# microscopic-image-analysis/DiffPointRasterisation.jl

Hardware: AMD Instinct MI355X
Metric: M points/s fwd+bwd, 10M pts→256³ grid; HBM GB/s vs roofline (higher is better)
Workload: dtype f32

## Files before the change

diffpointrasterisation.jl_amd/csrc/dpr_tiled.hip:

```cpp
#include <hip/hip_runtime.h>

#include <cstring>
#include <mutex>
#include <set>
#include <type_traits>
#include <utility>

#include "dpr_tiled_impl.h"

namespace dpr {

template <int NO>
__device__ __forceinline__ int primary_tile(const int (&ref0)[NO], const TileGeom<NO>& tg) {
    int t = 0, stride = 1;
    bool in = true;
#pragma unroll
    for (int d = 0; d < NO; ++d) {
        const int r = ref0[d] < 0 ? 0 : ref0[d];
        int c = r / TileDims<NO>::T[d];
        if (d == NO - 1) {
            c -= tg.tz0;
            in = (unsigned)c < (unsigned)tg.nt[d];
        }
        t += c * stride;
// ... 506 lines not shown
    __syncthreads();
    const Pose<T, NI, NO> ps = load_pose<T, NI, NO>(rot, trans, nullptr, b);
    const int64_t lo = (int64_t)slice * chunk;
    const int64_t hi = (lo + chunk < P) ? lo + chunk : P;
    if (lo >= hi) return;
    uint32_t wkey = 0;
    int64_t p = lo + threadIdx.x;
    T nxt[NI], nxt_w = T(1);
    {
        const int64_t pl = p < hi ? p : hi - 1;
        load_point<T, NI>(points, pl, nxt);
        if (HAS_PW) nxt_w = pw[pl];
    }
#pragma unroll
    for (int j = 0; j < NI; ++j) pin_value(nxt[j]);
    if (HAS_PW) pin_value(nxt_w);
    drain_vmem();
    while (p < hi) {
        T pt[NI];
#pragma unroll
        for (int j = 0; j < NI; ++j) pt[j] = nxt[j];
        const T w = nxt_w;
        const int64_t pc = p;
        p += kBinThreads;
        {
            const int64_t pl = p < hi ? p : hi - 1;
            load_point<T, NI>(points, pl, nxt);
            if (HAS_PW) nxt_w = pw[pl];
        }
        int ref0[NO];
        T dlo[NO];
        bool valid = ref_and_deltas<T, NI, NO>(pt, ps, gd, ref0, dlo);
        const int tl = valid ? primary_tile<NO>(ref0, tg) : -1;
        valid = tl >= 0;
        uint32_t pos = (uint32_t)P;
        if (valid) pos = atomicAdd(&cursor[tl], 1u);
        if (HAS_PW && valid) wkey = wrange_merge(wkey, abs_key(w));
        Rec4<T> r;
#pragma unroll
        for (int j = 0; j < 3; ++j) r.v[j] = (j < NI) ? pt[(j < NI) ? j : 0] : T(0);
        r.v[3] = HAS_PW ? w : idx_to_slot((uint32_t)pc, T(0));
        rec[pos] = r;
        if (HAS_PW && WANT_IDX) rec_idx[pos] = (uint32_t)pc;
        if (WANT_IDX) slot_of[pc] = pos;
        if (zero_dropped && !valid) {
#pragma unroll
            for (int j = 0; j < NI; ++j) ds_dpoints[pc * NI + j] = T(0);
            if (ds_dpw) ds_dpw[pc] = T(0);
        }
    }
    if (HAS_PW) publish_max_abs(maxpw, wkey);
}

template <typename T, int NI, int NO, bool HAS_PW, int S, bool GROUP, bool W3>
__global__ __launch_bounds__(kWcThreads) void k_scatter_wc(
    GridDesc<NO> gd, TileGeom<NO> tg, int64_t P, int64_t chunk, const T* __restrict__ points,
    const T* __restrict__ pw, const T* __restrict__ rot, const T* __restrict__ trans, int64_t b0,
    int nb, const uint32_t* __restrict__ prefix, const uint32_t* __restrict__ tile_start,
    RecT<T, W3>* __restrict__ rec, uint32_t* __restrict__ slot_of, T* __restrict__ ds_dpoints,
    T* __restrict__ ds_dpw, int zero_dropped, uint32_t* __restrict__ maxpw, int fused_scan,
    TileScanArgs ts) {
    const unsigned n_slices = fused_scan ? gridDim.x - 1u : gridDim.x;
    if (fused_scan && blockIdx.x == n_slices) {
        tilescan_body(ts.totals, ts.NT, ts.cap, ts.tile_start, ts.items, ts.n_items, ts.tile_parts,
                      ts.tile_slab, ts.split_list, ts.n_split, ts.hdr, ts.hdr_out, ts.rot,
                      ts.rot_words, ts.trans, ts.trans_words, ts.nonzero_bins, ts.nblk);
        return;
    }
    static_assert(!(W3 && HAS_PW), "compact records carry no point weight");
    constexpr int PPT = S / kWcThreads;
    uint32_t wkey = 0;
    if (!GROUP) nb = 1;
    const int NT = tg.NT, NTe = NT * nb;
    const uint32_t Pe = (uint32_t)(P * nb);
    extern __shared__ uint32_t dyn[];
    uint32_t* cursor = dyn;
    uint32_t* lhist = dyn + NTe;
    __shared__ RecT<T, W3> recs[S];
    __shared__ uint32_t dest[S];
    uint32_t* const wsum = dest;
    static_assert(S >= kWcThreads / kWave, "wave sums fit");
    const unsigned slice = xcd_slice(blockIdx.x, n_slices);
    const uint32_t* row = prefix + (size_t)slice * NTe;
    constexpr int kMaxBpt = 4096 / kWcThreads;
    const int lane = threadIdx.x & (kWave - 1), wave = threadIdx.x / kWave;
    if (fused_scan) {
        const int bpe = (NTe + kWcThreads - 1) / kWcThreads;
        const int e0 = threadIdx.x * bpe;
        uint32_t c[kMaxBpt], rw[kMaxBpt], sum = 0;
#pragma unroll
        for (int q = 0; q < kMaxBpt; ++q) {
            const int i = e0 + q;
            const bool in = q < bpe && i < NTe;
            c[q] = in ? ts.totals[i] : 0u;
            rw[q] = in ? row[i] : 0u;
            sum += c[q];
        }
        uint32_t incl = sum;
#pragma unroll
        for (int o = 1; o < kWave; o <<= 1) {
            const uint32_t v = __shfl_up(incl, o, kWave);
            if (lane >= o) incl += v;
        }
        if (lane == kWave - 1) wsum[wave] = incl;
        __syncthreads();
        uint32_t run = incl - sum;
        for (int wv = 0; wv < wave; ++wv) run += wsum[wv];
#pragma unroll
        for (int q = 0; q < kMaxBpt; ++q) {
            const int i = e0 + q;
            if (q < bpe && i < NTe) cursor[i] = run + rw[q];
            run += c[q];
        }
    } else {
        for (int i = threadIdx.x; i < NTe; i += kWcThreads) cursor[i] = tile_start[i] + row[i];
    }
    for (int i = threadIdx.x; i < NT; i += kWcThreads) lhist[i] = 0;
    __syncthreads();
    const int64_t lo = (int64_t)slice * chunk;
    const int64_t hi = (lo + chunk < P) ? lo + chunk : P;
    const int bpt = (NT + kWcThreads - 1) / kWcThreads;
    const int bin0 = threadIdx.x * bpt;
    if (lo >= hi) return;
    constexpr bool kPrefetch = !GROUP;
    auto load_sub = [&](int64_t sbase, T (&dp)[PPT][NI], T (&dw)[PPT]) {
        const int64_t left = hi - sbase;
        const uint32_t n = left >= S ? (uint32_t)S : (left > 0 ? (uint32_t)left : 0u);
        const T* const pb = points + (n ? sbase : hi - 1) * NI;
        const T* const wb = HAS_PW ? pw + (n ? sbase : hi - 1) : nullptr;
#pragma unroll
        for (int k = 0; k < PPT; ++k) {
            const uint32_t lp = threadIdx.x + (uint32_t)k * kWcThreads;
// ... 27 lines not shown
#pragma unroll
            for (int k = 0; k < PPT; ++k) {
                const uint32_t lp = threadIdx.x + (uint32_t)k * kWcThreads;
                int ref0[NO];
                T dlo[NO];
                bool valid = ref_and_deltas<T, NI, NO>(pt[k], ps, gd, ref0, dlo) && lp < nloc;
                tile[k] = valid ? primary_tile<NO>(ref0, tg) : -1;
                valid = tile[k] >= 0;
                lrank[k] = 0;
                if (valid) lrank[k] = atomicAdd(&lhist[tile[k]], 1u);
                if (HAS_PW && valid) wkey = wrange_merge(wkey, abs_key(w[k]));
            }
            lds_barrier();
            uint32_t cnt_sum = 0;
            uint32_t cnt[kMaxBpt];
#pragma unroll
            for (int q = 0; q < kMaxBpt; ++q) {
                const int i = bin0 + q;
                cnt[q] = (q < bpt && i < NT) ? lhist[i] : 0u;
                cnt_sum += cnt[q];
            }
            uint32_t incl = cnt_sum;
#pragma unroll
            for (int o = 1; o < kWave; o <<= 1) {
                const uint32_t v = __shfl_up(incl, o, kWave);
                if (lane >= o) incl += v;
            }
            if (lane == kWave - 1) wsum[wave] = incl;
            lds_barrier();
            uint32_t run = incl - cnt_sum;
            for (int wv = 0; wv < wave; ++wv) run += wsum[wv];
            uint32_t n_valid = 0;
#pragma unroll
            for (int wv = 0; wv < kWcThreads / kWave; ++wv) n_valid += wsum[wv];
#pragma unroll
            for (int q = 0; q < kMaxBpt; ++q) {
                const int i = bin0 + q;
                if (q < bpt && i < NT) lhist[i] = run;
                run += cnt[q];
            }
            lds_barrier();
#pragma unroll
            for (int k = 0; k < PPT; ++k) {
                const uint32_t lp = threadIdx.x + (uint32_t)k * kWcThreads;
                if (tile[k] >= 0) {
                    const uint32_t sidx = lhist[tile[k]] + lrank[k];
                    const uint32_t d = cur[tile[k]] + lrank[k];
                    RecT<T, W3> r;
#pragma unroll
                    for (int j = 0; j < 3; ++j) r.v[j] = (j < NI) ? pt[k][(j < NI) ? j : 0] : T(0);
                    if constexpr (!W3) r.v[3] = HAS_PW ? w[k] : idx_to_slot((uint32_t)base + lp, T(0));
                    recs[sidx] = r;
                    dest[sidx] = d;
                    if (slot_b) __builtin_nontemporal_store(d, &slot_b[lp]);
                } else if (lp < nloc) {
                    if (slot_b) __builtin_nontemporal_store(Pe, &slot_b[lp]);
                    if (zero_dropped) {
                        T* const dp_b = ds_dpoints + base * NI;
#pragma unroll
                        for (int j = 0; j < NI; ++j) dp_b[lp * NI + j] = T(0);
                        if (ds_dpw) (ds_dpw + base)[lp] = T(0);
                    }
                }
            }
            lds_barrier();
            for (uint32_t i = threadIdx.x; i < n_valid; i += kWcThreads) rec[dest[i]] = recs[i];
#pragma unroll
            for (int q = 0; q < kMaxBpt; ++q) {
                const int i = bin0 + q;
                if (q < bpt && i < NT) {
                    cur[i] += cnt[q];
                    lhist[i] = 0;
                }
            }
            lds_barrier();
        }
    }
    if (HAS_PW) publish_max_abs(maxpw, wkey);
}

struct LocalBinArgs {
    char* ws;
    size_t pose_stride;
    size_t off_rec, off_slot, off_desc, off_bdesc, off_ltot;
};
constexpr int kTouchCap = 1024;
template <typename T, int NI, int NO, bool HAS_PW, int S, bool W3, bool ONE, int TH, bool STAGE>
__global__ __launch_bounds__(TH, ((sizeof(T) == 4 && ONE) ? 8 : 4)) void k_bin_local(
    GridDesc<NO> gd, TileGeom<NO> tg, int64_t P, const T* __restrict__ points,
    const T* __restrict__ pw, const T* __restrict__ rot, const T* __restrict__ trans, int64_t b0,
    int nb, LocalBinArgs la, int want_slot, uint32_t spare_slot, T* __restrict__ ds_dpoints,
    T* __restrict__ ds_dpw, int zero_dropped) {
    static_assert(!(W3 && HAS_PW), "compact records carry no point weight");
    constexpr int PPT = S / TH;
    if (ONE) nb = 1;
    const int NT = tg.NT;
    extern __shared__ uint32_t lhist[];
    __shared__ RecT<T, W3> recs[STAGE ? S : 1];
    __shared__ uint16_t touched[kTouchCap];
    __shared__ uint32_t wsum[TH / kWave];
    __shared__ uint32_t s_ntouch, s_nvalid;
    for (int i = threadIdx.x; i < NT; i += TH) lhist[i] = 0;
    if (threadIdx.x == 0) s_ntouch = 0;
    const int64_t base = (int64_t)blockIdx.x * S;
    const uint32_t nloc = (uint32_t)((P - base < S) ? P - base : S);
    const T* const pts_blk = points + base * NI;
    const T* const pw_blk = HAS_PW ? pw + base : nullptr;
    T pt[PPT][NI], w[PPT];
#pragma unroll
    for (int k = 0; k < PPT; ++k) {
        const uint32_t lp = threadIdx.x + (uint32_t)k * TH;
        const uint32_t ll = lp < nloc ? lp : nloc - 1;
        if (nloc) {
            load_point<T, NI>(pts_blk, (int64_t)ll, pt[k]);
            w[k] = HAS_PW ? pw_blk[ll] : T(1);
        } else {
#pragma unroll
            for (int j = 0; j < NI; ++j) pt[k][j] = T(0);
            w[k] = T(1);
        }
    }
    if constexpr (HAS_PW) {
        uint32_t wkey = 0;
#pragma unroll
        for (int k = 0; k < PPT; ++k)
            if (threadIdx.x + (uint32_t)k * TH < nloc) wkey = wrange_merge(wkey, abs_key(w[k]));
        publish_max_abs((uint32_t*)(la.ws + la.off_ltot) + 2 * NT, wkey);
    }
    __syncthreads();
    const int lane = threadIdx.x & (kWave - 1), wave = threadIdx.x / kWave;
#pragma unroll 1
// ... 1698 lines not shown
    if (stale) {
        const T nan = T(__builtin_nanf(""));
        const int64_t b0 = (int64_t)ublock * (kUPB * 1024) + threadIdx.x;
#pragma unroll
        for (int k = 0; k < kUPB; ++k) {
            const int64_t p = b0 + k * 1024;
            if (p >= P) continue;
#pragma unroll
            for (int j = 0; j < NI; ++j) ds_dpoints[p * NI + j] = nan;
            if (ds_dpw) ds_dpw[p] = nan;
        }
        return;
    }
    const int64_t base = (int64_t)xcd_slice(ublock, ublocks) * (kUPB * 1024) + threadIdx.x;
    uint32_t slot[kUPB];
#pragma unroll
    for (int k = 0; k < kUPB; ++k) {
        const int64_t p = base + k * 1024;
        slot[k] = __builtin_nontemporal_load(&slot_of[p < P ? p : P - 1]);
    }
    Rec4<T> g[kUPB];
#pragma unroll
    for (int k = 0; k < kUPB; ++k) g[k] = grad[slot[k]];
    for (int j = 1; j < nb; ++j) {
        const Rec4<T>* gradj =
            pose_stride ? (const Rec4<T>*)((const char*)grad + (size_t)j * pose_stride) : grad;
        const uint32_t* slotj = pose_stride
                                    ? (const uint32_t*)((const char*)slot_of + (size_t)j * pose_stride)
                                    : slot_of + (size_t)j * P;
#pragma unroll
        for (int k = 0; k < kUPB; ++k) {
            const int64_t p = base + k * 1024;
            const Rec4<T> gj = gradj[slotj[p < P ? p : P - 1]];
#pragma unroll
            for (int c = 0; c < 4; ++c) g[k].v[c] += gj.v[c];
        }
    }
#pragma unroll
    for (int k = 0; k < kUPB; ++k) {
        const int64_t p = base + k * 1024;
        if (p >= P) continue;
        if (FIRST_POSE) {
#pragma unroll
            for (int j = 0; j < NI; ++j) __builtin_nontemporal_store(g[k].v[j], &ds_dpoints[p * NI + j]);
            if (ds_dpw) __builtin_nontemporal_store(g[k].v[3], &ds_dpw[p]);
        } else {
#pragma unroll
            for (int j = 0; j < NI; ++j) ds_dpoints[p * NI + j] += g[k].v[j];
            if (ds_dpw) ds_dpw[p] += g[k].v[3];
        }
    }
}

template <typename T>
__global__ __launch_bounds__(1024) void k_pose_reduce(PoseReduceArgs<T> pr) {
    pose_reduce_body<T>((int)blockIdx.x, blockIdx.y, gridDim.y > 1, pr);
}

template <typename T, int NI>
__global__ __launch_bounds__(256) void k_unsort(int64_t P, const uint32_t* __restrict__ inv_perm,
                                                const T* __restrict__ dp_sorted,
                                                const T* __restrict__ dpw_sorted,
                                                T* __restrict__ ds_dpoints, T* __restrict__ ds_dpw,
                                                const BinHeader* __restrict__ hdr) {
    constexpr int PER = 4;
    const int64_t q0 = (int64_t)blockIdx.x * (256 * PER) + threadIdx.x;
    if (hdr && hdr->verdict != 1u) {
        const T nan = T(__builtin_nanf(""));
#pragma unroll
        for (int k = 0; k < PER; ++k) {
            const int64_t q = q0 + k * 256;
            if (q >= P) continue;
#pragma unroll
            for (int j = 0; j < NI; ++j) ds_dpoints[q * NI + j] = nan;
            if (ds_dpw) ds_dpw[q] = nan;
        }
        return;
    }
    size_t i[PER];
#pragma unroll
    for (int k = 0; k < PER; ++k) {
        const int64_t q = q0 + k * 256;
        const size_t v = inv_perm[q < P ? q : P - 1];
        i[k] = v < (size_t)P ? v : 0;
    }
    T v[PER][NI], w[PER];
#pragma unroll
    for (int k = 0; k < PER; ++k) {
#pragma unroll
        for (int j = 0; j < NI; ++j) v[k][j] = dp_sorted[i[k] * NI + j];
        w[k] = ds_dpw ? dpw_sorted[i[k]] : T(0);
    }
#pragma unroll
    for (int k = 0; k < PER; ++k) {
        const int64_t q = q0 + k * 256;
        if (q >= P) continue;
#pragma unroll
        for (int j = 0; j < NI; ++j) ds_dpoints[q * NI + j] = v[k][j];
        if (ds_dpw) ds_dpw[q] = w[k];
    }
}

static int cu_count() {
    static std::mutex mu;
    static int cus[64] = {0};
    int dev = 0;
// ... 41 lines not shown
        while (nb * 2 <= pl.bg && b + nb * 2 <= B) nb *= 2;
        return nb;
    }
    int64_t copy_of(int64_t b) const { return kept && B > 1 ? b : (pl.local ? b % pl.lb : 0); }
    PoseWs at(int64_t b) const { return {ws + (size_t)copy_of(b) * pl.pose_stride, pl}; }
    bool opens_local_batch(int64_t b) const { return b % pl.lb == 0; }
    int local_batch(int64_t b) const { return (int)((B - b < pl.lb) ? B - b : pl.lb); }
};

template <typename K> static int allow_dynamic_lds(K kernel, size_t bytes, int max_bytes) {
    if (bytes <= 48 * 1024) return DPR_OK;
    static std::mutex mu;
    static std::set<std::pair<const void*, int>> done;
    int dev = 0;
    DPR_HIP(hipGetDevice(&dev));
    std::lock_guard<std::mutex> lock(mu);
    if (done.count({(const void*)kernel, dev})) return DPR_OK;
    DPR_HIP(hipFuncSetAttribute((const void*)kernel, hipFuncAttributeMaxDynamicSharedMemorySize, max_bytes));
    done.insert({(const void*)kernel, dev});
    return DPR_OK;
}


static bool scatter_is_wc(int NT, int nb) { return NT * nb <= 4096; }

static bool records_are_compact(int NT, int nb, bool has_pw, bool want_idx) {
    return !has_pw && !want_idx && scatter_is_wc(NT, nb);
}

template <typename T, int NI, int NO, bool HAS_PW, bool WANT_IDX>
static int launch_scatter(hipStream_t st, const GridDesc<NO>& gd, const TileGeom<NO>& tg,
                          const Plan& pl, const PoseWs& w, int64_t P, const T* points, const T* pw,
                          const T* rot, const T* trans, int64_t b, int nb, const TileScanArgs& ts,
                          bool fused) {
    if (scatter_is_wc(tg.NT, nb)) {
        constexpr int S = (sizeof(T) == 4) ? kWcPpt * kWcThreads : kWcPpt * kWcThreads / 2;
        const size_t lds2 = (size_t)tg.NT * (nb + 1) * 4;
#define DPR_LAUNCH_WC(GROUP, W3)                                                                  \
    hipLaunchKernelGGL((k_scatter_wc<T, NI, NO, HAS_PW, S, GROUP, W3>),                          \
                       dim3(pl.nblk + (fused ? 1 : 0)),                                          \
                       dim3(kWcThreads), lds2, st, gd, tg, P, pl.chunk, points, pw, rot, trans, \
                       b, nb, w.counts(), w.tile_start(),      \
                       w.rec<RecT<T, W3>>(),                                                     \
                       WANT_IDX ? w.slot() : (uint32_t*)nullptr,                                 \
                       (T*)nullptr, (T*)nullptr, 0, w.weight_keys(), fused ? 1 : 0, ts)
        if constexpr (!HAS_PW) {
            if (records_are_compact(tg.NT, nb, false, WANT_IDX)) {
                if (nb > 1) DPR_LAUNCH_WC(true, true);
                else DPR_LAUNCH_WC(false, true);
                return DPR_OK;
            }
        }
        if (nb > 1) DPR_LAUNCH_WC(true, false);
        else DPR_LAUNCH_WC(false, false);
#undef DPR_LAUNCH_WC
        return DPR_OK;
    }
    const size_t lds = (size_t)tg.NT * 4;
    if (int rc = allow_dynamic_lds(k_scatter<T, NI, NO, HAS_PW, WANT_IDX>, lds, kMaxTiles * 4)) return rc;
    hipLaunchKernelGGL((k_scatter<T, NI, NO, HAS_PW, WANT_IDX>), dim3(pl.nblk), dim3(kBinThreads),
                       lds, st, gd, tg, P, pl.chunk, points, pw, rot, trans, b,
                       w.counts(), w.tile_start(), w.rec<Rec4<T>>(),
                       w.idx(), w.slot(), (T*)nullptr, (T*)nullptr, 0, w.weight_keys());
    return DPR_OK;
}

template <typename T, int NI, int NO, typename Args>
static void fill_header(Args& a, const GridDesc<NO>& gd, const Plan& pl, int64_t P, const T* points, const T* pw,
                        const T* hdr_points, const T* hdr_pw, const T* rot, const T* trans, int64_t b,
                        bool keep_valid) {
    if (!hdr_points) {
        hdr_points = points;
        hdr_pw = pw;
    }
    int64_t grid64[3] = {1, 1, 1};
    for (int d = 0; d < NO; ++d) grid64[d] = gd.n[d];
    a.hdr = make_header<T, NI, NO>(grid64, P, hdr_points, hdr_pw);
    a.hdr.state = keep_valid ? kBinValid : 0u;
    a.hdr.layout = plan_layout_id(pl);
    a.rot = (const uint32_t*)(rot + b * (NO * NI));
    a.rot_words = (int)(NO * NI * sizeof(T) / 4);
    a.trans = (const uint32_t*)(trans + b * NO);
    a.trans_words = (int)(NO * sizeof(T) / 4);
}

template <typename T, int NI, int NO>
static int bin_points(hipStream_t st, const GridDesc<NO>& gd, const TileGeom<NO>& tg,
                      const Plan& pl, char* ws, int64_t P, const T* points, const T* pw,
                      const T* rot, const T* trans, int64_t b, int nb, bool want_idx,
                      bool keep_valid, const T* hdr_points, const T* hdr_pw) {
    const PoseWs w{ws, pl};
    const int NTe = tg.NT * nb;
    const size_t lds = (size_t)NTe * 4;
    if (nb > 1) {
        if (int rc = allow_dynamic_lds(k_count<T, NI, NO, true>, lds, kMaxTiles * 4)) return rc;
        hipLaunchKernelGGL((k_count<T, NI, NO, true>), dim3(pl.nblk), dim3(kBinThreads), lds, st,
                           gd, tg, P, pl.chunk, points, rot, trans, b, nb, w.counts(), w.nzbins());
    } else {
        if (int rc = allow_dynamic_lds(k_count<T, NI, NO, false>, lds, kMaxTiles * 4)) return rc;
        hipLaunchKernelGGL((k_count<T, NI, NO, false>), dim3(pl.nblk), dim3(kBinThreads), lds, st,
                           gd, tg, P, pl.chunk, points, rot, trans, b, nb, w.counts(), w.nzbins());
    }
    stage_mark(st);
    TileScanArgs ts;
    ts.totals = w.totals();
    ts.NT = NTe;
// ... 234 lines not shown
        pr.NT = tg.NT;
        pr.n_in = NI;
        pr.n_out = NO;
        pr.b0 = b;
        pr.ds_drotation = d_rot;
        pr.ds_dtranslation = d_trans;
        pr.ds_dbackground = d_bg;
        pr.ds_dout_weight = d_ow;
        pr.loss = rs.target ? rs.loss : nullptr;
        pr.hdr = hdr;
        pr.accumulate = slab > 0 ? 1 : 0;
        const unsigned n_reduce = (unsigned)(rs.target ? NVAL + 1 : NVAL);
        bool reduced = false;
        if (reuse || (pl.local && !walk.opens_local_batch(b))) {
            stage_mark(st);
            stage_mark(st);
            stage_mark(st);
        } else if (pl.local) {
            if (int rc = bin_points_local<T, NI, NO>(st, gd, tg, pl, w.base, P, points, pw, rot, trans, b,
                                                     walk.local_batch(b), true, false, user_points, user_pw))
                return rc;
        } else if (int rc = bin_points<T, NI, NO>(st, gd, tg, pl, w.base, P, points, pw, rot, trans, b,
                                                  (int)nb, true, false, user_points, user_pw))
            return rc;
#define DPR_LAUNCH_GATHER_RUNS(HAS_PW)                                                           \
    hipLaunchKernelGGL((k_tile_gather_runs<T, NI, NO, HAS_PW, true, true, true>),                \
                       dim3(pl.max_items), dim3(gather_threads<T>()), 0, st, gd, tg,             \
                       w.rec<Rec4<T>>(), w.sdesc(), pl.nsub * pl.sub, w.idx(), w.items(),        \
                       w.n_items(), pl.max_items, g, rot, trans, ow, b, d_pts, d_pw, partials,   \
                       rs, want, hdr)
#define DPR_LAUNCH_GATHER_PLAIN(HAS_PW)                                                          \
    hipLaunchKernelGGL((k_tile_gather<T, NI, NO, HAS_PW, true, true>), dim3(pl.max_items),       \
                       dim3(gather_threads<T>()), 0, st, gd, tg, w.rec<Rec4<T>>(), P * nb,       \
                       w.idx(), w.items(), w.n_items(), pl.max_items, g, rot, trans, ow, b,      \
                       d_pts, d_pw, partials, rs, want, hdr)
        if (pl.local) {
            if (pw) DPR_LAUNCH_GATHER_RUNS(true);
            else DPR_LAUNCH_GATHER_RUNS(false);
        } else if (pw) DPR_LAUNCH_GATHER_PLAIN(true);
        else DPR_LAUNCH_GATHER_PLAIN(false);
#undef DPR_LAUNCH_GATHER_RUNS
#undef DPR_LAUNCH_GATHER_PLAIN
        stage_mark(st);
        if (P > 0) {
#define DPR_LAUNCH_UNPERM(FIRST, UPB, RB)                                                        \
    hipLaunchKernelGGL((k_unpermute<T, NI, FIRST, UPB>),                                         \
                       dim3((unsigned)((P + UPB * 1024 - 1) / (UPB * 1024)) + (RB)), dim3(1024), \
                       0, st, P, (int)nb, w.rec<const Rec4<T>>(), w.slot(), d_pts, d_pw,         \
                       (const BinHeader*)hdr, (int)(RB), pr, (size_t)0)
            if (batch_unperm) {
            } else if (nb > 1) {
                if (first_acc) DPR_LAUNCH_UNPERM(true, 1, 0);
                else DPR_LAUNCH_UNPERM(false, 1, 0);
            } else {
                if (first_acc) DPR_LAUNCH_UNPERM(true, kUpb, n_reduce);
                else DPR_LAUNCH_UNPERM(false, kUpb, n_reduce);
                reduced = true;
            }
#undef DPR_LAUNCH_UNPERM
        }
        stage_mark(st);
        if (!reduced)
            hipLaunchKernelGGL((k_pose_reduce<T>), dim3(n_reduce, (unsigned)nb), dim3(1024), 0, st,
                               pr);
        stage_mark(st);
        }
        if (batch_unperm && ((b + 1) % ub == 0 || b + 1 == B)) {
            const int64_t bs = b - b % ub;
            const PoseWs wu = walk.at(bs);
            const BinHeader* uh = reuse ? wu.hdr() : (const BinHeader*)nullptr;
            PoseReduceArgs<T> none{};
            auto unpermute_batch = bs == 0 ? k_unpermute<T, NI, true, 1> : k_unpermute<T, NI, false, 1>;
            hipLaunchKernelGGL(unpermute_batch, dim3((unsigned)((P + 1023) / 1024)), dim3(1024), 0, st, P,
                               (int)(b + 1 - bs), wu.rec<const Rec4<T>>(), wu.slot(), d_pts, d_pw, uh, 0, none,
                               pl.pose_stride);
        }
    }
    if (pl.sort_inside && P > 0)
        hipLaunchKernelGGL((k_unsort<T, NI>), dim3((unsigned)((P + 1023) / 1024)), dim3(256), 0, st, P,
                           (const uint32_t*)(ws + pl.off_iperm), (const T*)d_pts, (const T*)d_pw,
                           d_pts_user, d_pw_user,
                           reuse ? (const BinHeader*)(ws + pl.off_hdr) : (const BinHeader*)nullptr);
    DPR_HIP(hipGetLastError());
    return DPR_OK;
}


template <typename T>
__global__ __launch_bounds__(256) void k_channel_weights(int64_t P, int C, const T* __restrict__ pw,
                                                        const Rec4<T>* __restrict__ rec,
                                                        const uint32_t* __restrict__ n_rec,
                                                        T* __restrict__ w_sorted, int64_t plane,
                                                        uint32_t* __restrict__ keys) {
    uint32_t key[kMaxChannels];
#pragma unroll
    for (int c = 0; c < kMaxChannels; ++c) key[c] = 0;
    const int64_t n = *n_rec;
    for (int64_t r = (int64_t)blockIdx.x * 256 + threadIdx.x; r < n; r += (int64_t)gridDim.x * 256) {
        uint32_t idx = slot_to_idx(rec[r].v[3]);
        idx = idx < (uint64_t)P ? idx : 0u;
#pragma unroll
        for (int c = 0; c < kMaxChannels; ++c) {
            if (c < C) {
                const T w = pw[(int64_t)idx * C + c];
                w_sorted[(int64_t)c * plane + r] = w;
                key[c] = wrange_merge(key[c], abs_key(w));
// ... 211 lines not shown
```

diffpointrasterisation.jl_amd/csrc/dpr_tiled_impl.h:

```cpp
#pragma once
#include <hip/hip_runtime.h>

#include "../../include/dpr.h"
#include "dpr_device.h"
#include "dpr_jvp.h"
#include "dpr_tiled.h"

namespace dpr {

template <int NO> struct TileDims;
template <> struct TileDims<3> {
    static constexpr int T[3] = {64, 16, 8};
};
template <> struct TileDims<2> {
    static constexpr int T[3] = {32, 32, 1};
};
constexpr int kMaxTiles = 32768;
constexpr int kBinThreads = 1024;
constexpr int kWcThreads = 1024;
constexpr int kWcPpt = 4;
constexpr int kSplatThreads = 512;
constexpr int kSplatRunsOcc = 4;
template <typename T> __host__ __device__ constexpr int gather_threads() {
    return sizeof(T) == 8 ? 512 : 256;
// ... 8 lines not shown

template <int NO> struct TileGeom {
    int nt[NO];
    int NT;
    int tz0;
    int ghost;
};

template <int NO> __host__ __device__ constexpr int tile_voxels() {
    int v = 1;
    for (int d = 0; d < NO; ++d) v *= TileDims<NO>::T[d];
    return v;
}
template <int NO> __host__ __device__ constexpr int tile_voxels_halo() {
    int v = 1;
    for (int d = 0; d < NO; ++d) v *= TileDims<NO>::T[d] + 1;
    return v;
}
template <int NO> __host__ __device__ constexpr int halo_count() {
    return tile_voxels_halo<NO>() - tile_voxels<NO>();
}

struct SlabCut {
    int per_layer, layers, lps, nslab;
};

constexpr uint32_t kBinMagic = 0x44505242u, kBinValid = 1u;
struct alignas(16) BinHeader {
    uint32_t magic, state;
    uint32_t elem, n_in, n_out, has_pw;
    int64_t P;
    int32_t grid[3];
    uint32_t verdict;
    uint64_t points, pw;
    uint32_t layout, pad_[3];
    unsigned char pose[96];
};

struct alignas(16) WorkItem {
    uint32_t tile, begin, end;
    uint32_t part_nparts;
};

struct alignas(8) RunDesc {
    uint32_t start;
    uint32_t tile_count;
    __host__ __device__ uint32_t tile() const { return tile_count & 0x7fffu; }
    __host__ __device__ uint32_t count() const { return tile_count >> 15; }
};
constexpr int kMaxLocalTiles = 16384;
constexpr int kMaxRuns = 256;
constexpr int kMaxRunsGather = 64;

struct Plan {
    int bg;
    int nblk;
    int64_t chunk;
    uint32_t cap;
    int max_items;
    int max_slabs;
    size_t off_hdr, off_counts, off_totals, off_tile_start, off_items, off_nitems, off_nzbins, off_tparts, off_tslab,
        off_split, off_rec, off_idx, off_slot, off_aux, total;
    bool sort_inside;
    size_t off_spts, off_spw, off_perm, off_iperm, off_sgrad, off_sgradw, off_sorttmp;
    size_t pose_stride;
    bool local;
    int lb;
    int64_t copies;
    int sub;
    int64_t nsub;
    int64_t max_desc;
    size_t off_ltot, off_dstart, off_dcursor, off_bdesc, off_desc, off_sdesc;
};

template <int NO> bool make_slab_cut(const int64_t* grid, SlabCut* sc);
template <int NO> TileGeom<NO> slab_geom(const int64_t* grid, const SlabCut& sc, int s, bool forward);
int slab_max_tiles(const SlabCut& sc);

struct PlanRequest {
    size_t elem;
    int n_in, n_out;
    int tiles;
    int64_t P, B;
    int max_group;
    bool coherent;
    bool share_batch;
    bool slabbed;
    bool fwd_only;
};
PlanRequest plan_request(size_t elem, int op, unsigned flags, int n_in, int n_out, const SlabCut& sc, int64_t P,
                         int64_t B);
Plan make_plan(const PlanRequest& rq);
Plan pose_plan(size_t elem, int n_in, int n_out, const SlabCut& sc, int64_t P);
uint32_t plan_layout_id(const Plan& pl);
int tiled_check(int n_out, const int64_t* grid, int64_t P, unsigned flags, const char* binning_flag, SlabCut* sc);
bool pose_binning_cut(int n_out, const int64_t* grid, int64_t P, SlabCut* sc);
size_t channel_part_bytes(size_t elem, int64_t P, int C);
size_t jvp_part_bytes(size_t elem, int64_t P);

size_t coarse_workspace_bytes(size_t elem, int64_t P);

}
```

diffpointrasterisation.jl_amd/csrc/dpr_tiled_plan.hip:

```cpp
#include <cstdlib>

#include "dpr_tiled_impl.h"

namespace dpr {

static int max_tiles() {
    static const int v = [] {
        const char* e = getenv("DPR_MAX_TILES");
        int x = e ? atoi(e) : kMaxTiles;
        return x < 16 ? 16 : (x > kMaxTiles ? kMaxTiles : x);
    }();
    return v;
}
template <int NO> bool make_slab_cut(const int64_t* grid, SlabCut* sc) {
    const int cap = max_tiles();
    int64_t per = 1;
    for (int d = 0; d + 1 < NO; ++d) per *= (grid[d] + TileDims<NO>::T[d] - 1) / TileDims<NO>::T[d];
    const int64_t layers = (grid[NO - 1] + TileDims<NO>::T[NO - 1] - 1) / TileDims<NO>::T[NO - 1];
    if (per > cap / 2 || layers > (1 << 20)) return false;
    sc->per_layer = (int)per;
    sc->layers = (int)layers;
    if (per * layers <= cap) {
        sc->lps = (int)layers;
        sc->nslab = 1;
// ... 84 lines not shown
            pl.lb = B < 16 ? (int)B : 16;
        } else {
            pl.lb = B < 8 ? (int)B : 8;
            while (pl.lb > 1 && P1 * pl.lb > ((int64_t)1 << 29)) --pl.lb;
        }
    }
    pl.copies = share_batch ? B : pl.lb;
    const int NT = NT1 * pl.bg;
    const int64_t P = P1 * pl.bg;
    int64_t nblk, chunk;
    if (NT <= 4096) {
        const int64_t sub = (elem == 4) ? kWcPpt * kWcThreads : kWcPpt * kWcThreads / 2;
        chunk = ((P1 + 255) / 256 + sub - 1) / sub * sub;
        if (chunk < sub) chunk = sub;
    } else {
        nblk = (P1 + 8191) / 8192;
        if (nblk < 1) nblk = 1;
        if (nblk > kMaxBinBlocks) nblk = kMaxBinBlocks;
        chunk = (P1 + nblk - 1) / nblk;
        chunk = (chunk + kBinThreads - 1) / kBinThreads * kBinThreads;
        if (chunk < kBinThreads) chunk = kBinThreads;
    }
    nblk = (P1 + chunk - 1) / chunk;
    if (nblk < 1) nblk = 1;
    pl.nblk = (int)nblk;
    pl.chunk = chunk;
    size_t o = 0;
    auto take = [&o](size_t bytes) {
        const size_t at = o;
        o += align_up(bytes);
        return at;
    };
    pl.off_hdr = take(sizeof(BinHeader));
    pl.off_counts = take((size_t)nblk * NT * 4);
    pl.off_totals = take((size_t)NT * 4);
    pl.off_tile_start = take((size_t)(NT + 1) * 4);
    int64_t cap = P / 256;
    const int64_t cap_min = fwd_only ? 2 * 4096 : 4096;
    if (cap < cap_min) cap = cap_min;
    if (n_out == 2) {
        cap = P / 2048;
        if (cap < 2048) cap = 2048;
    }
    pl.cap = (uint32_t)cap;
    pl.max_slabs = (int)(2 * ((P + cap - 1) / cap) + 1);
    pl.max_items = NT + pl.max_slabs;
    pl.off_items = take((size_t)pl.max_items * sizeof(WorkItem));
    pl.off_nitems = take(4);
    pl.off_nzbins = take((size_t)kMaxBinBlocks * 4);
    pl.off_tparts = take((size_t)NT * 4);
    pl.off_tslab = take((size_t)NT * 4);
    pl.off_split = take((size_t)(pl.max_slabs / 2 + 2) * 4);
    pl.sub = elem == 4 ? 4096 : 2048;
    pl.nsub = (P1 + pl.sub - 1) / pl.sub;
    if (pl.nsub < 1) pl.nsub = 1;
    pl.max_desc = 0;
    int64_t nrec = P;
    if (pl.local) {
        pl.max_desc = pl.nsub * pl.sub;
        nrec = pl.nsub * pl.sub;
        pl.off_ltot = take((size_t)(2 * NT1 + 2) * 4);
        pl.off_dcursor = take((size_t)NT1 * 4);
        pl.off_dstart = take((size_t)(NT1 + 1) * 4);
        pl.off_bdesc = take((size_t)pl.nsub * 4);
        pl.off_desc = take((size_t)pl.max_desc * sizeof(RunDesc));
        pl.off_sdesc = take((size_t)pl.max_desc * sizeof(RunDesc));
    }
    pl.off_rec = take((size_t)(nrec + 1) * 4 * elem);
    pl.off_idx = take((size_t)(P1 + 1) * 4);
    pl.off_slot = take((size_t)(P + 1) * 4);
    if (pl.copies > 1) {
        pl.pose_stride = o;
        o += (size_t)(pl.copies - 1) * pl.pose_stride;
    }
    pl.off_spts = pl.off_spw = pl.off_perm = pl.off_iperm = pl.off_sgrad = pl.off_sgradw = pl.off_sorttmp = o;
    if (pl.sort_inside) {
        pl.off_spts = take((size_t)P1 * n_in * elem);
        pl.off_spw = take((size_t)P1 * elem);
        pl.off_perm = o;
        pl.off_iperm = take((size_t)P1 * 4);
        pl.off_sgrad = take((size_t)P1 * n_in * elem);
        pl.off_sgradw = take((size_t)P1 * elem);
        pl.off_sorttmp = take(coarse_workspace_bytes(elem, P1));
    }
    pl.off_aux = o;
    const size_t nvh = (n_out == 3) ? tile_voxels_halo<3>() : tile_voxels_halo<2>();
    const size_t halo = align_up((size_t)NT * ((n_out == 3) ? halo_count<3>() : halo_count<2>()) * elem) +
                        align_up((size_t)pl.max_slabs * nvh * elem);
    const size_t partials = (size_t)pl.max_items * 16 * 8;
    o += align_up(halo > partials ? halo : partials);
    pl.total = o;
    return pl;
}

uint32_t plan_layout_id(const Plan& pl) {
    uint64_t h = 1469598103934665603ull;
    auto mix = [&](uint64_t v) {
        for (int i = 0; i < 8; ++i) {
            h ^= (v >> (8 * i)) & 0xffu;
            h *= 1099511628211ull;
        }
    };
    mix(pl.local ? 1 : 0);
    mix((uint64_t)pl.bg);
    mix((uint64_t)pl.sub);
    mix((uint64_t)pl.cap);
    mix(pl.off_items);
    mix(pl.off_rec);
    mix(pl.off_idx);
    mix(pl.off_slot);
    mix(pl.off_aux);
    mix(pl.local ? pl.off_sdesc : 0);
    mix(pl.pose_stride);
    mix(pl.off_iperm);
    mix((uint64_t)pl.lb);
    const uint32_t id = (uint32_t)(h ^ (h >> 32));
    return id ? id : 1u;
}

static bool grid_cut(int n_out, const int64_t* grid, SlabCut* sc) {
    return n_out == 3 ? make_slab_cut<3>(grid, sc) : make_slab_cut<2>(grid, sc);
}

bool tiled_supported(int n_out, const int64_t* grid) {
    SlabCut sc;
    return grid_cut(n_out, grid, &sc);
}

int tiled_slabs(int n_out, const int64_t* grid) {
    SlabCut sc;
    return grid_cut(n_out, grid, &sc) ? sc.nslab : 0;
}

bool tiled_preferred(int op, int n_out, const int64_t* grid, int64_t P, int64_t B, int64_t G) {
    (void)G;
    if (P >= (int64_t)1 << 32) return false;
    SlabCut sc;
    if (!grid_cut(n_out, grid, &sc)) return false;
    const int64_t NT_all = (int64_t)sc.per_layer * sc.layers;
    const int64_t per_tile = op == DPR_OP_RASTER ? (n_out == 3 ? 60 : 48)
                                                 : (n_out == 3 ? 320 : (NT_all <= 4096 ? 150 : 430));
    if (P < per_tile * NT_all) return false;
    if (sc.nslab > 1) {
        return op == DPR_OP_RASTER && P >= 1000000;
    }
    const int NT = sc.per_layer * sc.layers;
    const bool grouped = B >= 4 && pose_group(NT, P, B, 0) >= 4;
    if (op == DPR_OP_RASTER && B < 4 && (NT <= 64 || (n_out == 3 && NT <= 256))) return P >= 100000;
    if (op == DPR_OP_RASTER) return P >= (grouped ? 60000 : 250000);
    if (B >= 4) return P >= (grouped ? 300000 : 600000);
    return P >= 250000;
}

int tiled_tiles(int n_out, const int64_t* grid) {
    SlabCut sc;
    return grid_cut(n_out, grid, &sc) ? slab_max_tiles(sc) : -1;
}

bool tiled_batch_share_ok(int n_out, const int64_t* grid, int64_t P, int64_t B) {
    if (B < 2 || P < 1 || P * B > ((int64_t)1 << 29)) return false;
    SlabCut sc;
    if (!grid_cut(n_out, grid, &sc) || sc.nslab != 1) return false;
    return sc.per_layer * sc.layers * 2 > 4096;
}

int tiled_check(int n_out, const int64_t* grid, int64_t P, unsigned flags, const char* binning_flag, SlabCut* sc) {
    const bool quiet = !binning_flag;
    if (!grid_cut(n_out, grid, sc))
// ... 57 lines not shown
```

Baseline: 27140.

## Add run-ordered slot map so unpermute gathers sorted gradients coalesced

In the single-pose, non-local write-combined scatter, the slot map is now written in sorted (destination) order together with a uint16 local point index, instead of scattering one slot per point. A new unpermute kernel reads these run-ordered slots, so gradient records are gathered in near-sequential order. It then permutes them in LDS back to point order and writes coalesced point gradients. It also fuses the pose reduction into the same launch. The cost is an extra uint16 array per point and an extra LDS staging buffer, and the new path only applies when its plan conditions hold.

```diff
diff --git a/diffpointrasterisation.jl_amd/csrc/dpr_tiled.hip b/diffpointrasterisation.jl_amd/csrc/dpr_tiled.hip
--- a/diffpointrasterisation.jl_amd/csrc/dpr_tiled.hip
+++ b/diffpointrasterisation.jl_amd/csrc/dpr_tiled.hip
@@ -582,14 +582,14 @@
     if (HAS_PW) publish_max_abs(maxpw, wkey);
 }
 
-template <typename T, int NI, int NO, bool HAS_PW, int S, bool GROUP, bool W3>
-__global__ __launch_bounds__(kWcThreads) void k_scatter_wc(
-    GridDesc<NO> gd, TileGeom<NO> tg, int64_t P, int64_t chunk, const T* __restrict__ points,
+template <typename T, int NI, int NO, bool HAS_PW, int S, bool GROUP, bool W3, bool RUNS>
+__device__ __forceinline__ void scatter_wc_body(
+    const GridDesc<NO>& gd, const TileGeom<NO>& tg, int64_t P, int64_t chunk, const T* __restrict__ points,
     const T* __restrict__ pw, const T* __restrict__ rot, const T* __restrict__ trans, int64_t b0,
     int nb, const uint32_t* __restrict__ prefix, const uint32_t* __restrict__ tile_start,
-    RecT<T, W3>* __restrict__ rec, uint32_t* __restrict__ slot_of, T* __restrict__ ds_dpoints,
-    T* __restrict__ ds_dpw, int zero_dropped, uint32_t* __restrict__ maxpw, int fused_scan,
-    TileScanArgs ts) {
+    RecT<T, W3>* __restrict__ rec, uint32_t* __restrict__ slot_of, uint16_t* __restrict__ run_lp,
+    T* __restrict__ ds_dpoints, T* __restrict__ ds_dpw, int zero_dropped, uint32_t* __restrict__ maxpw,
+    int fused_scan, const TileScanArgs& ts) {
     const unsigned n_slices = fused_scan ? gridDim.x - 1u : gridDim.x;
     if (fused_scan && blockIdx.x == n_slices) {
         tilescan_body(ts.totals, ts.NT, ts.cap, ts.tile_start, ts.items, ts.n_items, ts.tile_parts,
@@ -598,6 +598,7 @@
         return;
     }
     static_assert(!(W3 && HAS_PW), "compact records carry no point weight");
+    static_assert(!RUNS || (!GROUP && !W3 && S <= 65536), "the sorted map: one pose, 4-word records, uint16 owners");
     constexpr int PPT = S / kWcThreads;
     uint32_t wkey = 0;
     if (!GROUP) nb = 1;
@@ -608,6 +609,7 @@
     uint32_t* lhist = dyn + NTe;
     __shared__ RecT<T, W3> recs[S];
     __shared__ uint32_t dest[S];
+    __shared__ uint16_t lpos[RUNS ? S : 1];
     uint32_t* const wsum = dest;
     static_assert(S >= kWcThreads / kWave, "wave sums fit");
     const unsigned slice = xcd_slice(blockIdx.x, n_slices);
@@ -741,9 +743,10 @@
                     if constexpr (!W3) r.v[3] = HAS_PW ? w[k] : idx_to_slot((uint32_t)base + lp, T(0));
                     recs[sidx] = r;
                     dest[sidx] = d;
-                    if (slot_b) __builtin_nontemporal_store(d, &slot_b[lp]);
+                    if constexpr (RUNS) lpos[sidx] = (uint16_t)lp;
+                    else if (slot_b) __builtin_nontemporal_store(d, &slot_b[lp]);
                 } else if (lp < nloc) {
-                    if (slot_b) __builtin_nontemporal_store(Pe, &slot_b[lp]);
+                    if (!RUNS && slot_b) __builtin_nontemporal_store(Pe, &slot_b[lp]);
                     if (zero_dropped) {
                         T* const dp_b = ds_dpoints + base * NI;
 #pragma unroll
@@ -753,7 +756,20 @@
                 }
             }
             lds_barrier();
-            for (uint32_t i = threadIdx.x; i < n_valid; i += kWcThreads) rec[dest[i]] = recs[i];
+            if constexpr (RUNS) {
+                uint16_t* const lp_b = run_lp + base;
+                for (uint32_t i = threadIdx.x; i < nloc; i += kWcThreads) {
+                    const bool owned = i < n_valid;
+                    const uint32_t d = dest[i];
+                    if (owned) {
+                        rec[d] = recs[i];
+                        __builtin_nontemporal_store(lpos[i], &lp_b[i]);
+                    }
+                    __builtin_nontemporal_store(owned ? d : kRunEnd, &slot_b[i]);
+                }
+            } else {
+                for (uint32_t i = threadIdx.x; i < n_valid; i += kWcThreads) rec[dest[i]] = recs[i];
+            }
 #pragma unroll
             for (int q = 0; q < kMaxBpt; ++q) {
                 const int i = bin0 + q;
@@ -766,6 +782,29 @@
         }
     }
     if (HAS_PW) publish_max_abs(maxpw, wkey);
+}
+template <typename T, int NI, int NO, bool HAS_PW, int S, bool GROUP, bool W3>
+__global__ __launch_bounds__(kWcThreads) void k_scatter_wc(
+    GridDesc<NO> gd, TileGeom<NO> tg, int64_t P, int64_t chunk, const T* __restrict__ points,
+    const T* __restrict__ pw, const T* __restrict__ rot, const T* __restrict__ trans, int64_t b0,
+    int nb, const uint32_t* __restrict__ prefix, const uint32_t* __restrict__ tile_start,
+    RecT<T, W3>* __restrict__ rec, uint32_t* __restrict__ slot_of, T* __restrict__ ds_dpoints,
+    T* __restrict__ ds_dpw, int zero_dropped, uint32_t* __restrict__ maxpw, int fused_scan,
+    TileScanArgs ts) {
+    scatter_wc_body<T, NI, NO, HAS_PW, S, GROUP, W3, false>(gd, tg, P, chunk, points, pw, rot, trans, b0, nb, prefix,
+                                                            tile_start, rec, slot_of, nullptr, ds_dpoints, ds_dpw,
+                                                            zero_dropped, maxpw, fused_scan, ts);
+}
+template <typename T, int NI, int NO, bool HAS_PW, int S>
+__global__ __launch_bounds__(kWcThreads) void k_scatter_wc_runs(
+    GridDesc<NO> gd, TileGeom<NO> tg, int64_t P, int64_t chunk, const T* __restrict__ points,
+    const T* __restrict__ pw, const T* __restrict__ rot, const T* __restrict__ trans, int64_t b0,
+    const uint32_t* __restrict__ prefix, const uint32_t* __restrict__ tile_start, Rec4<T>* __restrict__ rec,
+    uint32_t* __restrict__ run_slot, uint16_t* __restrict__ run_lp, uint32_t* __restrict__ maxpw, int fused_scan,
+    TileScanArgs ts) {
+    scatter_wc_body<T, NI, NO, HAS_PW, S, false, false, true>(gd, tg, P, chunk, points, pw, rot, trans, b0, 1, prefix,
+                                                              tile_start, rec, run_slot, run_lp, nullptr, nullptr, 0,
+                                                              maxpw, fused_scan, ts);
 }
 
 struct LocalBinArgs {
@@ -2570,6 +2609,79 @@
     }
 }
 
+template <typename T, int NI, bool FIRST_POSE>
+__global__ __launch_bounds__(1024, 8) void k_unpermute_runs(int64_t P, const Rec4<T>* __restrict__ grad,
+                                                            const uint32_t* __restrict__ run_slot,
+                                                            const uint16_t* __restrict__ run_lp,
+                                                            T* __restrict__ ds_dpoints, T* __restrict__ ds_dpw,
+                                                            const BinHeader* __restrict__ hdr,
+                                                            int reduce_blocks, PoseReduceArgs<T> pr) {
+    constexpr int S = sizeof(T) == 4 ? kWcPpt * kWcThreads : kWcPpt * kWcThreads / 2;
+    constexpr int PPT = S / 1024;
+    __shared__ Rec4<T> stage[S];
+    if ((int)blockIdx.x < reduce_blocks) {
+        pose_reduce_body<T>((int)blockIdx.x, 0u, false, pr);
+        return;
+    }
+    const unsigned ublock = blockIdx.x - (unsigned)reduce_blocks;
+    const unsigned ublocks = gridDim.x - (unsigned)reduce_blocks;
+    if (hdr && hdr->verdict != 1u) {
+        const T nan = T(__builtin_nanf(""));
+        const int64_t b0 = (int64_t)ublock * S + threadIdx.x;
+#pragma unroll
+        for (int k = 0; k < PPT; ++k) {
+            const int64_t p = b0 + k * 1024;
+            if (p >= P) continue;
+#pragma unroll
+            for (int j = 0; j < NI; ++j) ds_dpoints[p * NI + j] = nan;
+            if (ds_dpw) ds_dpw[p] = nan;
+        }
+        return;
+    }
+    const int64_t base = (int64_t)xcd_slice(ublock, ublocks) * S;
+    const uint32_t nloc = (uint32_t)((P - base < S) ? P - base : S);
+    uint32_t slot[PPT], lp[PPT];
+#pragma unroll
+    for (int k = 0; k < PPT; ++k) {
+        const uint32_t i = threadIdx.x + (uint32_t)k * 1024;
+        const uint32_t ic = i < nloc ? i : nloc - 1;
+        slot[k] = __builtin_nontemporal_load(&run_slot[base + ic]);
+        lp[k] = __builtin_nontemporal_load(&run_lp[base + ic]);
+        if (i >= nloc) slot[k] = kRunEnd;
+    }
+    Rec4<T> zero;
+#pragma unroll
+    for (int c = 0; c < 4; ++c) zero.v[c] = T(0);
+#pragma unroll
+    for (int k = 0; k < PPT; ++k) stage[threadIdx.x + k * 1024] = zero;
+    Rec4<T> g[PPT];
+#pragma unroll
+    for (int k = 0; k < PPT; ++k) {
+        g[k] = zero;
+        if (slot[k] < (uint64_t)P) g[k] = grad[slot[k]];
+    }
+    __syncthreads();
+#pragma unroll
+    for (int k = 0; k < PPT; ++k)
+        if (slot[k] < (uint64_t)P) stage[lp[k] & (uint32_t)(S - 1)] = g[k];
+    __syncthreads();
+    const T* const words = &stage[0].v[0];
+    T* const dp = ds_dpoints + base * NI;
+    for (uint32_t e = threadIdx.x; e < nloc * NI; e += 1024) {
+        const T v = words[(e / NI) * 4 + e % NI];
+        if (FIRST_POSE) __builtin_nontemporal_store(v, &dp[e]);
+        else dp[e] += v;
+    }
+    if (ds_dpw) {
+        T* const dw = ds_dpw + base;
+        for (uint32_t q = threadIdx.x; q < nloc; q += 1024) {
+            const T v = stage[q].v[3];
+            if (FIRST_POSE) __builtin_nontemporal_store(v, &dw[q]);
+            else dw[q] += v;
+        }
+    }
+}
+
 template <typename T>
 __global__ __launch_bounds__(1024) void k_pose_reduce(PoseReduceArgs<T> pr) {
     pose_reduce_body<T>((int)blockIdx.x, blockIdx.y, gridDim.y > 1, pr);
@@ -2717,6 +2829,11 @@
             }
         }
         if (nb > 1) DPR_LAUNCH_WC(true, false);
+        else if (WANT_IDX && pl.run_map)
+            hipLaunchKernelGGL((k_scatter_wc_runs<T, NI, NO, HAS_PW, S>), dim3(pl.nblk + (fused ? 1 : 0)),
+                               dim3(kWcThreads), lds2, st, gd, tg, P, pl.chunk, points, pw, rot, trans, b, w.counts(),
+                               w.tile_start(), w.rec<Rec4<T>>(), w.slot(), (uint16_t*)w.idx(), w.weight_keys(),
+                               fused ? 1 : 0, ts);
         else DPR_LAUNCH_WC(false, false);
 #undef DPR_LAUNCH_WC
         return DPR_OK;
@@ -3057,6 +3174,12 @@
             } else if (nb > 1) {
                 if (first_acc) DPR_LAUNCH_UNPERM(true, 1, 0);
                 else DPR_LAUNCH_UNPERM(false, 1, 0);
+            } else if (pl.run_map) {
+                auto unpermute_runs = first_acc ? k_unpermute_runs<T, NI, true> : k_unpermute_runs<T, NI, false>;
+                hipLaunchKernelGGL(unpermute_runs, dim3((unsigned)((P + pl.sub - 1) / pl.sub) + n_reduce), dim3(1024),
+                                   0, st, P, w.rec<const Rec4<T>>(), (const uint32_t*)w.slot(),
+                                   (const uint16_t*)w.idx(), d_pts, d_pw, (const BinHeader*)hdr, (int)n_reduce, pr);
+                reduced = true;
             } else {
                 if (first_acc) DPR_LAUNCH_UNPERM(true, kUpb, n_reduce);
                 else DPR_LAUNCH_UNPERM(false, kUpb, n_reduce);
diff --git a/diffpointrasterisation.jl_amd/csrc/dpr_tiled_impl.h b/diffpointrasterisation.jl_amd/csrc/dpr_tiled_impl.h
--- a/diffpointrasterisation.jl_amd/csrc/dpr_tiled_impl.h
+++ b/diffpointrasterisation.jl_amd/csrc/dpr_tiled_impl.h
@@ -84,6 +84,7 @@
 constexpr int kMaxRuns = 256;
 constexpr int kMaxRunsGather = 64;
 
+constexpr uint32_t kRunEnd = 0xffffffffu;
 struct Plan {
     int bg;
     int nblk;
@@ -91,6 +92,7 @@
     uint32_t cap;
     int max_items;
     int max_slabs;
+    bool run_map;
     size_t off_hdr, off_counts, off_totals, off_tile_start, off_items, off_nitems, off_nzbins, off_tparts, off_tslab,
         off_split, off_rec, off_idx, off_slot, off_aux, total;
     bool sort_inside;
diff --git a/diffpointrasterisation.jl_amd/csrc/dpr_tiled_plan.hip b/diffpointrasterisation.jl_amd/csrc/dpr_tiled_plan.hip
--- a/diffpointrasterisation.jl_amd/csrc/dpr_tiled_plan.hip
+++ b/diffpointrasterisation.jl_amd/csrc/dpr_tiled_plan.hip
@@ -160,6 +160,7 @@
     pl.off_tslab = take((size_t)NT * 4);
     pl.off_split = take((size_t)(pl.max_slabs / 2 + 2) * 4);
     pl.sub = elem == 4 ? 4096 : 2048;
+    pl.run_map = pl.bg == 1 && !pl.local && NT1 <= 4096 && pl.copies == 1;
     pl.nsub = (P1 + pl.sub - 1) / pl.sub;
     if (pl.nsub < 1) pl.nsub = 1;
     pl.max_desc = 0;
@@ -222,6 +223,7 @@
     mix(pl.pose_stride);
     mix(pl.off_iperm);
     mix((uint64_t)pl.lb);
+    mix(pl.run_map ? 1 : 0);
     const uint32_t id = (uint32_t)(h ^ (h >> 32));
     return id ? id : 1u;
 }
```

After: 28270 (median of 6 runs). 1.04x the previous value.
